# madsjulia/GeostatInversion.jl

Measured on AMD Instinct MI355X. Metric: randSVD GB/s + top-k singular-value rel-err, n=1e6 rank=256, higher is better.
Workload: dtype f64

## Files before the change

### geostatinversion.jl_amd/build.py

```python
import os
import shutil
import subprocess
import sys
from concurrent.futures import ThreadPoolExecutor

HERE = os.path.dirname(os.path.abspath(__file__))
CSRC = os.path.join(HERE, "csrc")
OBJ = os.path.join(HERE, "build")
LIB = os.path.join(HERE, "libgsi_hip.so")
SOURCES = ["gemm_f64.hip", "gemm_f64_gen1.hip", "syrk_f64.hip", "panel_lu_leaf.hip", "panel_lu_blocks.hip", "panel_lu_streamed.hip", "panel_lu_sharded.hip", "panel_qr.hip", "cholqr.hip", "lowrank_power.hip", "jacobi_svd.hip", "misc.hip", "lsqr_dev.hip", "block_cg.hip", "block_pcg.hip", "block_slq.hip", "pivoted_chol.hip", "pointcov_gemm.hip", "fft_cov.hip", "fft_gridcov_plan.hip", "fftrf_sample.hip", "fftrf_interp.hip", "interp_adjoint.hip", "gridcov_sample.hip","pcga_forward.hip", "fwd_adjoint.hip", "chol_saddle.hip", "posterior_var.hip", "posterior_exact.hip",
           "hip_backend.hip", "hip_backend_products.hip", "hip_backend_sampler.hip", "hip_backend_panels.hip", "hip_backend_lowrank.hip", "hip_backend_pcga.hip",
           "hip_comm.hip", "pipeline.cpp", "solvers.cpp", "pcga.cpp", "api.cpp"]
HEADERS = ["backend.hpp", "hip_backend.hpp", "hip_backend_impl.hpp", "hip_common.hpp", "panel_lu_dev.hpp", "pipeline.hpp", "solvers.hpp", "pcga.hpp", "lsqr_state.hpp", "cg_state.hpp", "block_cg_host.hpp", "slq_state.hpp", "pchol_state.hpp", "pivoted_chol_host.hpp", "pointcov.hpp", "pointcov_gen.hpp", "host_staging.hpp", "gemm_f64_kernel.inc.hpp", "fft_line.hpp", "jacobi_sched.hpp", "fwd_plan.hpp", "fwd_adjoint_plan.hpp", "fwd_adjoint_host.hpp", "fftrf_points.hpp", "interp_adjoint_plan.hpp", "saddle_host.hpp", "posterior_host.hpp", "posterior_exact_host.hpp", "../../include/gsi_hip.h"]
CXXFLAGS = ["-O3", "-std=c++17", "-fPIC", "--offload-arch=gfx950", "-Wall", "-Wno-unused-function",
            "-Wno-unused-result", "-Wno-unused-value"]
RESOURCE_FLAG = "-Rpass-analysis=kernel-resource-usage"
_RES_KEYS = {"TotalSGPRs": "sgprs", "VGPRs": "vgprs", "AGPRs": "agprs", "ScratchSize [bytes/lane]": "scratch_bytes_per_lane",
             "Occupancy [waves/SIMD]": "occupancy_waves_per_simd", "SGPRs Spill": "sgpr_spills", "VGPRs Spill": "vgpr_spills",
             "LDS Size [bytes/block]": "lds_bytes_per_block", "Dynamic Stack": "dynamic_stack"}


def parse_resource_remarks(text):
    out, cur = {}, None
    for line in text.splitlines():
        if "remark:" not in line or "[-Rpass-analysis=kernel-resource-usage]" not in line:
            continue
        body = line.split("remark:", 1)[1].replace("[-Rpass-analysis=kernel-resource-usage]", "").strip()
        if ":" not in body:
            continue
        key, val = [x.strip() for x in body.rsplit(":", 1)]
        if key == "Function Name":
            cur = out.setdefault(val, {})
        elif cur is not None and key in _RES_KEYS:
            cur[_RES_KEYS[key]] = (val == "True") if key == "Dynamic Stack" else int(val)
    return out


def hipcc_version():
    r = subprocess.run([_hipcc(), "--version"], capture_output=True, text=True)
    lines = [ln.strip() for ln in r.stdout.splitlines() if ln.strip()]
    return "; ".join(lines[:2])


def kernel_resources():
    import json
    res = {}
    for src in SOURCES:
        if not src.endswith(".hip"):
            continue
        path = os.path.join(OBJ, src.replace(".", "_") + ".resources.json")
        if not os.path.exists(path):
            raise RuntimeError(f"{path} missing: run build() (it recompiles sources whose resource record is absent)")
        for name, r in json.load(open(path)).items():
            res[name] = dict(r, source=src)
    return res


def _hipcc():
    for cand in (shutil.which("hipcc"), "/opt/rocm/bin/hipcc"):
        if cand and os.path.exists(cand):
            return cand
    raise RuntimeError("hipcc not found: libgsi_hip.so cannot be built (there is no CPU fallback)")


def _newer(target, deps):
    if not os.path.exists(target):
# ... 52 lines not shown
```

### geostatinversion.jl_amd/csrc/cholqr.hip

```cpp
#include "hip_common.hpp"
#include <atomic>
#include <cfloat>
#include <cstdio>
#include <cstdlib>

namespace gsi { namespace hipk {

constexpr int CQ_TB = 32;

__global__ __launch_bounds__(256) void cq_diagmax_kernel(const double* __restrict__ G, int l, double* __restrict__ tiny) {
  __shared__ double s[256];
  double mx = 0.0;
  for (int i = threadIdx.x; i < l; i += 256) mx = fmax(mx, G[i + (int64_t)i * l]);
  s[threadIdx.x] = mx;
  __syncthreads();
  for (int st = 128; st > 0; st >>= 1) {
    if (threadIdx.x < st) s[threadIdx.x] = fmax(s[threadIdx.x], s[threadIdx.x + st]);
    __syncthreads();
  }
  if (threadIdx.x == 0) tiny[0] = s[0] * (double)l * DBL_EPSILON * 16.0;
}

__device__ __forceinline__ double cq_bcast(double v, int src) {
  const int lo = __builtin_amdgcn_readlane(__double2loint(v), src);
  const int hi = __builtin_amdgcn_readlane(__double2hiint(v), src);
  return __hiloint2double(hi, lo);
}

__global__ __launch_bounds__(256) void cq_chol_block_kernel(double* __restrict__ G, int l, int j0, int b,
                                                            const double* __restrict__ tiny_p,
                                                            double* __restrict__ Xout ,
                                                            int32_t* __restrict__ flag) {
  __shared__ double X[CQ_TB][CQ_TB + 1];
  const int tid = threadIdx.x;
  if (tid < 64) {
    const double tiny = tiny_p[0];
    const int c = tid & (CQ_TB - 1);
    double col[CQ_TB], x[CQ_TB];
#pragma unroll
    for (int r = 0; r < CQ_TB; ++r)
      col[r] = (r < b && c < b) ? G[(j0 + r) + (int64_t)(j0 + c) * l] : (r == c ? 1.0 : 0.0);
    bool bad = false;
#pragma unroll
    for (int k = 0; k < CQ_TB; ++k) {
      double d = cq_bcast(col[k], k);
      if (k < b && !(d > tiny)) { bad = true; d = 1.0; }
      const double ukk = sqrt(d);
      col[k] = (c == k) ? ukk : col[k] / ukk;
#pragma unroll
      for (int r = k + 1; r < CQ_TB; ++r) col[r] -= cq_bcast(col[k], r) * col[k];
      __builtin_amdgcn_sched_barrier(0);
    }
    if (bad && tid == 0) atomicOr(flag, 1);
#pragma unroll
    for (int r = CQ_TB - 1; r >= 0; --r) {
      double sacc = (r == c) ? 1.0 : 0.0;
#pragma unroll
      for (int p = r + 1; p < CQ_TB; ++p) sacc -= cq_bcast(col[r], p) * x[p];
      x[r] = (r <= c) ? sacc / cq_bcast(col[r], r) : 0.0;
      __builtin_amdgcn_sched_barrier(0);
    }
    if (tid < CQ_TB) {
#pragma unroll
      for (int r = 0; r < CQ_TB; ++r) {
        X[r][c] = x[r];
        Xout[r + c * CQ_TB] = x[r];
        if (r < b && c < b) G[(j0 + r) + (int64_t)(j0 + c) * l] = (r <= c) ? col[r] : 0.0;
      }
    }
  }
  __syncthreads();
  for (int c = j0 + b + tid; c < l; c += 256) {
    double g[CQ_TB];
#pragma unroll
    for (int r = 0; r < CQ_TB; ++r) g[r] = (r < b) ? G[(j0 + r) + (int64_t)c * l] : 0.0;
#pragma unroll 1
    for (int r = 0; r < b; ++r) {
      double s = 0.0;
#pragma unroll
      for (int p = 0; p < CQ_TB; ++p) s += X[p][r] * g[p];
// ... 11 lines not shown
  __shared__ double Xs[CQ_TB][CQ_TB + 1];
  __shared__ double xs[8][CQ_TB + 1];
  const int tid = threadIdx.x, c = tid & (CQ_TB - 1), rl = tid >> 5;
  for (int e = tid; e < CQ_TB * CQ_TB; e += 256) Xs[e & (CQ_TB - 1)][e >> 5] = X[e];
  for (int64_t r0 = (int64_t)blockIdx.x * 8; r0 < m; r0 += (int64_t)gridDim.x * 8) {
    const int64_t r = r0 + rl;
    __syncthreads();
    xs[rl][c] = (r < m && c < b) ? Y[r + (j0 + c) * ld] : 0.0;
    __syncthreads();
    double s = 0.0;
#pragma unroll
    for (int p = 0; p < CQ_TB; ++p) s += xs[rl][p] * Xs[p][c];
    if (r < m && c < b) Y[r + (j0 + c) * ld] = s;
  }
}

__global__ __launch_bounds__(256) void cq_orth_check_kernel(const double* __restrict__ G, int l, double thresh,
                                                            int32_t* __restrict__ flag) {
  const int64_t total = (int64_t)l * l;
  bool bad = false;
  for (int64_t e = (int64_t)blockIdx.x * 256 + threadIdx.x; e < total; e += (int64_t)gridDim.x * 256) {
    const int r = (int)(e % l), c = (int)(e / l);
    const double v = G[e] - (r == c ? 1.0 : 0.0);
    if (!(fabs(v) <= thresh)) bad = true;
  }
  if (bad) atomicOr(flag, 2);
}

__global__ void cq_mirror_upper_kernel(double* __restrict__ G, int l) {
  const int64_t total = (int64_t)l * l;
  for (int64_t e = (int64_t)blockIdx.x * blockDim.x + threadIdx.x; e < total; e += (int64_t)gridDim.x * blockDim.x) {
    const int r = (int)(e % l), c = (int)(e / l);
    if (r > c) G[e] = G[c + (int64_t)r * l];
  }
}

__global__ void cq_triprod_kernel(const double* __restrict__ R2, const double* __restrict__ R1, int l,
                                  double* __restrict__ R) {
  const int64_t total = (int64_t)l * l;
  for (int64_t e = (int64_t)blockIdx.x * blockDim.x + threadIdx.x; e < total;
       e += (int64_t)gridDim.x * blockDim.x) {
    const int r = (int)(e % l), c = (int)(e / l);
    double s = 0.0;
    if (r <= c)
      for (int p = r; p <= c; ++p) s += R2[r + (int64_t)p * l] * R1[p + (int64_t)c * l];
    R[e] = s;
  }
}

constexpr int CQF_THREADS = 512;
constexpr int CQF_MAXL = 384;
constexpr int CQF_LDU = CQF_MAXL - CQ_TB + 16;
constexpr int CQF_LDK = CQF_MAXL - CQ_TB + 4;
constexpr int CQF_DS = CQ_TB + 4;
static_assert(CQF_LDU % 32 == 16 && CQF_LDK % 32 == 4, "LDS strides");
typedef double cq_double4 __attribute__((ext_vector_type(4)));
constexpr size_t CQF_LDS_BYTES = sizeof(double) * ((size_t)CQ_TB * CQF_LDU + (size_t)CQ_TB * CQF_DS + 2 * CQ_TB + 64);

__device__ __forceinline__ void cqf_chol_diag(double* __restrict__ G, int l, int j0, int b, double tiny, double* __restrict__ Ds,
                                                        double* __restrict__ Dinv, int32_t* __restrict__ flag, int lane) {
  const int c = lane & (CQ_TB - 1);
  double col[CQ_TB];
#pragma unroll
  for (int r = 0; r < CQ_TB; ++r)
    col[r] = (r < b && c < b && r <= c) ? G[(j0 + r) + (int64_t)(j0 + c) * l] : (r == c ? 1.0 : 0.0);
  bool bad = false;
  double rdiag = 1.0;
#pragma unroll
  for (int k = 0; k < CQ_TB; ++k) {
    double d = cq_bcast(col[k], k);
    if (k < b && !(d > tiny)) { bad = true; d = 1.0; }
    double rs = __builtin_amdgcn_rsq(d);
    rs = rs * (1.5 - 0.5 * d * rs * rs);
    rs = rs * (1.5 - 0.5 * d * rs * rs);
    const double ukk = d * rs;
    col[k] = (c == k) ? ukk : col[k] * rs;
    if (c == k) rdiag = rs;
#pragma unroll
    for (int r = k + 1; r < CQ_TB; ++r) col[r] -= cq_bcast(col[k], r) * col[k];
    __builtin_amdgcn_sched_barrier(0);
  }
  if (bad && lane == 0) atomicOr(flag, 1);
  if (lane < CQ_TB) {
    Dinv[c] = rdiag;
#pragma unroll
    for (int r = 0; r < CQ_TB; ++r) {
      const double v = (r <= c) ? col[r] : 0.0;
      Ds[r * CQF_DS + c] = v;
      if (r < b && c < b) G[(j0 + r) + (int64_t)(j0 + c) * l] = v;
    }
  }
}
__device__ __forceinline__ void cqf_inv_diag(const double* __restrict__ G, int l, int j0, int b, double* __restrict__ X, int lane) {
  const int c = lane & (CQ_TB - 1);
  double col[CQ_TB], x[CQ_TB];
#pragma unroll
  for (int r = 0; r < CQ_TB; ++r)
    col[r] = (r < b && c < b && r <= c) ? G[(j0 + r) + (int64_t)(j0 + c) * l] : (r == c ? 1.0 : 0.0);
#pragma unroll
  for (int r = CQ_TB - 1; r >= 0; --r) {
    double sacc = (r == c) ? 1.0 : 0.0;
#pragma unroll
    for (int p = r + 1; p < CQ_TB; ++p) sacc -= cq_bcast(col[r], p) * x[p];
    x[r] = (r <= c) ? sacc / cq_bcast(col[r], r) : 0.0;
    __builtin_amdgcn_sched_barrier(0);
  }
  if (lane < CQ_TB && c < b) {
#pragma unroll
    for (int r = 0; r < CQ_TB; ++r)
      if (r < b) X[(j0 + r) + (int64_t)(j0 + c) * l] = x[r];
  }
}
template <bool VEC>
__device__ __forceinline__ void cqf_block_row_col(double* __restrict__ gcol , int b,
                                                  const double* __restrict__ Ds, const double* __restrict__ Dinv,
                                                  double* __restrict__ us ) {
  double g[CQ_TB];
  if constexpr (VEC) {
    const double2* g2 = reinterpret_cast<const double2*>(gcol);
#pragma unroll
    for (int p = 0; p < CQ_TB; p += 2) { const double2 v = g2[p >> 1]; g[p] = v.x; g[p + 1] = v.y; }
  } else {
#pragma unroll
    for (int p = 0; p < CQ_TB; ++p) g[p] = (p < b) ? gcol[p] : 0.0;
  }
#pragma unroll
  for (int pb = 0; pb < CQ_TB; pb += 8) {
    double acc[8];
#pragma unroll
    for (int j = 0; j < 8; ++j) acc[j] = g[pb + j];
#pragma unroll 4
    for (int q = 0; q < pb; ++q) {
      const double uq = us[q * CQF_LDU];
      const double* dr = Ds + q * CQF_DS + pb;
#pragma unroll
      for (int j = 0; j < 8; ++j) acc[j] -= dr[j] * uq;
    }
#pragma unroll
    for (int j = 0; j < 8; ++j) {
#pragma unroll
      for (int i = 0; i < j; ++i) acc[j] -= Ds[(pb + i) * CQF_DS + pb + j] * acc[i];
      acc[j] *= Dinv[pb + j];
    }
#pragma unroll
    for (int j = 0; j < 8; ++j) {
      const double v = (pb + j < b) ? acc[j] : 0.0;
      us[(pb + j) * CQF_LDU] = v;
      if constexpr (!VEC) { if (pb + j < b) gcol[pb + j] = v; }
    }
    if constexpr (VEC) {
      double2* o2 = reinterpret_cast<double2*>(gcol + pb);
#pragma unroll
      for (int j = 0; j < 8; j += 2) o2[j >> 1] = make_double2(acc[j], acc[j + 1]);
    }
    asm volatile("" ::: "memory");
  }
}
#define CQF_STAMP(ph) do { if (trace != nullptr && tid == 0) { const unsigned long long now_ = wall_clock64(); trace[ph] += now_ - t_last; t_last = now_; } } while (0)
__device__ __forceinline__ void cqf_tri_inverse(const double* __restrict__ G, int l, double* __restrict__ X, double* Us,
                                                double* Ds, int tid, int lane, int wave, unsigned long long* trace,
                                                unsigned long long& t_last);
__global__ __launch_bounds__(CQF_THREADS) void cq_chol_inv_kernel(double* __restrict__ G, int l, double* __restrict__ X,
                                                                  int32_t* __restrict__ flag, unsigned long long* __restrict__ trace,
                                                                  const int32_t* __restrict__ skip) {
  if (skip != nullptr && *skip != 0) return;
// ... 337 lines not shown
        phiT = diag ? 0.5 * t : t;
        q = diag ? di * di : accQ[jj] + (di + dJ[wave * CQS_NJ + jj]) * r1;
      }
      const double one = diag ? 1.0 : 0.0;
      rv = (one + r1) - phiT;
      xv = (one - r1) + (q + phiT);
    }
    G[i + (int64_t)j * l] = rv;
    X[i + (int64_t)j * l] = xv;
  }
}

static inline int grid_for(int64_t total, int cap = 2048) {
  int64_t g = (total + 255) / 256;
  if (g > cap) g = cap;
  if (g < 1) g = 1;
  return (int)g;
}

__global__ void cq_identity_kernel(double* __restrict__ X, int l) {
  const int64_t total = (int64_t)l * l;
  for (int64_t e = (int64_t)blockIdx.x * blockDim.x + threadIdx.x; e < total; e += (int64_t)gridDim.x * blockDim.x)
    X[e] = (e % l == e / l) ? 1.0 : 0.0;
}

__global__ __launch_bounds__(256) void cq_shift_kernel(double* __restrict__ G, int l, double m) {
  __shared__ double s[256], mx[256];
  double tr = 0.0, dm = 0.0;
  for (int i = threadIdx.x; i < l; i += 256) {
    const double g = G[i + (int64_t)i * l];
    tr += g;
    dm = fmax(dm, g);
  }
  s[threadIdx.x] = tr;
  mx[threadIdx.x] = dm;
  __syncthreads();
  for (int st = 128; st > 0; st >>= 1) {
    if (threadIdx.x < st) {
      s[threadIdx.x] += s[threadIdx.x + st];
      mx[threadIdx.x] = fmax(mx[threadIdx.x], mx[threadIdx.x + st]);
    }
    __syncthreads();
  }
  const double shift = fmax(4.0 * (double)l * sqrt(m) * (0.5 * DBL_EPSILON) * s[0], 4.0 * 16.0 * (double)l * DBL_EPSILON * mx[0]);
  for (int i = threadIdx.x; i < l; i += 256) G[i + (int64_t)i * l] += shift;
}

size_t cholqr_small_doubles(int64_t l) {
  const int64_t nblk = (l + CQ_TB - 1) / CQ_TB;
  return (size_t)(7 * l * l + nblk * CQ_TB * CQ_TB + 64);
}

namespace {
struct CqBufs { double *R1, *R2, *R3, *Gt, *X1, *X2, *X3, *Rinv; };
inline CqBufs cq_bufs(double* small, int l) {
  const size_t ll = (size_t)l * l;
  return {small, small + ll, small + 2 * ll, small + 3 * ll, small + 4 * ll, small + 5 * ll, small + 6 * ll,
          small + 7 * ll};
}

void cq_round(hipStream_t st, const double* src, int64_t lds, double* dst, int64_t ldd, int64_t m, int l, double* Rp,
              double* X, const CqBufs& b, bool check, int32_t* flag, double* gemm_ws, bool apply, bool shift = false) {
  const int nblk = (l + CQ_TB - 1) / CQ_TB;
  if (!syrk_full_from_upper(st, l, m, src, lds, Rp, l, gemm_ws)) {
    gemm_f64_syrk_upper(st, l, m, src, lds, Rp, l, gemm_ws);
    hipLaunchKernelGGL(cq_mirror_upper_kernel, dim3(64), dim3(256), 0, st, Rp, l);
  }
  if (check)
    hipLaunchKernelGGL(cq_orth_check_kernel, dim3(grid_for((int64_t)l * l, 64)), dim3(256), 0, st, Rp, l, 0.1, flag);
  if (shift) hipLaunchKernelGGL(cq_shift_kernel, dim3(1), dim3(256), 0, st, Rp, l, (double)m);
  static const bool fused_off = (getenv("GSI_CQ_FUSED") != nullptr && getenv("GSI_CQ_FUSED")[0] == '0');
  if (!fused_off && l <= CQF_MAXL && l >= 1) {
    static std::atomic<uint64_t> attr_mask{0};
    if (first_use_on_this_device(attr_mask))
      (void)hipFuncSetAttribute((const void*)cq_chol_inv_kernel, hipFuncAttributeMaxDynamicSharedMemorySize, (int)CQF_LDS_BYTES);
    static const bool trace_on = (getenv("GSI_CQ_TRACE") != nullptr);
    unsigned long long* trace = nullptr;
    if (trace_on && hipMalloc((void**)&trace, 8 * sizeof(unsigned long long)) == hipSuccess) hipMemsetAsync(trace, 0, 8 * sizeof(unsigned long long), st);
    hipLaunchKernelGGL(cq_chol_inv_kernel, dim3(1), dim3(CQF_THREADS), CQF_LDS_BYTES, st, Rp, l, X, flag, trace,
                       (const int32_t*)nullptr);
    if (trace != nullptr) {
      unsigned long long h[8];
      hipMemcpyAsync(h, trace, sizeof(h), hipMemcpyDeviceToHost, st);
      hipStreamSynchronize(st);
      hipFree(trace);
      fprintf(stderr, "[gsi cq trace] l = %d: set-up %.1f us, diagonal blocks %.1f, block rows %.1f, trailing updates %.1f, diagonal inverses %.1f, "
              "W rows %.1f, inverse tiles %.1f\n", l, h[0] / 100.0, h[1] / 100.0, h[2] / 100.0, h[3] / 100.0, h[4] / 100.0, h[5] / 100.0, h[6] / 100.0);
    }
    if (apply && !trmm_upper_tall(st, m, l, src, lds, X, l, dst, ldd))
      gemm_f64_trmm_upper(st, m, l, l, src, lds, X, l, dst, ldd, gemm_ws);
    return;
  }
  hipLaunchKernelGGL(cq_diagmax_kernel, dim3(1), dim3(256), 0, st, Rp, l, b.Gt);
  for (int jb = 0; jb < nblk; ++jb) {
    const int j0 = jb * CQ_TB;
    const int bb = (l - j0 < CQ_TB) ? (l - j0) : CQ_TB;
    hipLaunchKernelGGL(cq_chol_block_kernel, dim3(1), dim3(256), 0, st, Rp, l, j0, bb, b.Gt,
                       b.Rinv + (size_t)jb * CQ_TB * CQ_TB, flag);
    const int t = l - j0 - bb;
    if (t > 0)
      gemm_f64(st, true, t, t, bb, -1.0, Rp + j0 + (int64_t)(j0 + bb) * l, l, Rp + j0 + (int64_t)(j0 + bb) * l, l, 1.0,
               Rp + (j0 + bb) + (int64_t)(j0 + bb) * l, l, gemm_ws);
  }
  hipLaunchKernelGGL(cq_identity_kernel, dim3(grid_for((int64_t)l * l, 256)), dim3(256), 0, st, X, l);
  for (int jb = 0; jb < nblk; ++jb) {
    const int64_t j0 = (int64_t)jb * CQ_TB;
    const int bb = (int)((l - j0 < CQ_TB) ? (l - j0) : CQ_TB);
    if (j0 > 0)
      gemm_f64(st, false, j0 + bb, bb, j0, -1.0, X, l, Rp + j0 * (int64_t)l, l, 1.0, X + j0 * l, l, gemm_ws);
    hipLaunchKernelGGL(cq_right_mult_kernel, dim3((unsigned)((j0 + bb + 7) / 8)), dim3(256), 0, st, X, j0 + bb, (int64_t)l,
                       j0, bb, b.Rinv + (size_t)jb * CQ_TB * CQ_TB);
  }
  if (apply && !trmm_upper_tall(st, m, l, src, lds, X, l, dst, ldd))
    gemm_f64_trmm_upper(st, m, l, l, src, lds, X, l, dst, ldd, gemm_ws);
}
}

void cholqr2_factor(hipStream_t st, const double* Y, int64_t m, int64_t l64, int64_t ld, double* T, int64_t ldt,
                    double* small, int32_t* flag, double* gemm_ws) {
  const int l = (int)l64;
  const CqBufs b = cq_bufs(small, l);
  cq_round(st, Y, ld, T, ldt, m, l, b.R1, b.X1, b, false, flag, gemm_ws, true);
  cq_round(st, T, ldt, nullptr, 0, m, l, b.R2, b.X2, b, true, flag, gemm_ws, false);
}

void cholqr2_apply(hipStream_t st, double* Y, int64_t m, int64_t l64, int64_t ld, const double* T, int64_t ldt,
                   double* R, double* small, double* gemm_ws) {
  const int l = (int)l64;
  const CqBufs b = cq_bufs(small, l);
  if (!trmm_upper_tall(st, m, l, T, ldt, b.X2, l, Y, ld)) gemm_f64_trmm_upper(st, m, l, l, T, ldt, b.X2, l, Y, ld, gemm_ws);
  if (R != nullptr)
    hipLaunchKernelGGL(cq_triprod_kernel, dim3(grid_for((int64_t)l * l, 256)), dim3(256), 0, st, b.R2, b.R1, l, R);
}

void cholqr2_R(hipStream_t st, int64_t l64, double* small, double* R) {
  const int l = (int)l64;
  const CqBufs b = cq_bufs(small, l);
  hipLaunchKernelGGL(cq_triprod_kernel, dim3(grid_for((int64_t)l * l, 256)), dim3(256), 0, st, b.R2, b.R1, l, R);
}
const double* cholqr2_X2(const double* small, int64_t l) { return small + 5 * (size_t)l * (size_t)l; }

void mirror_upper(hipStream_t st, double* G, int64_t l) {
  hipLaunchKernelGGL(cq_mirror_upper_kernel, dim3(64), dim3(256), 0, st, G, (int)l);
}
bool cq_gram_round(hipStream_t st, double* Gm, int64_t l64, double* X, bool check, int32_t* flag, int32_t* series, double* tmp) {
  const int l = (int)l64;
  if (l < 1 || l > CQF_MAXL) return false;
  static const bool series_off = (getenv("GSI_CQ_SERIES") != nullptr && getenv("GSI_CQ_SERIES")[0] == '0');
  const bool by_series = check && !series_off && series != nullptr && tmp != nullptr;
  if (by_series) hipLaunchKernelGGL(cq_mirror_copy_kernel, dim3(64), dim3(256), 0, st, Gm, l, tmp);
  else hipLaunchKernelGGL(cq_mirror_upper_kernel, dim3(64), dim3(256), 0, st, Gm, l);
  if (check)
    hipLaunchKernelGGL(cq_orth_check_kernel, dim3(grid_for((int64_t)l * l, 64)), dim3(256), 0, st, Gm, l, 0.1, flag);
  if (by_series) {
    const int nb = (l + CQS_T - 1) / CQS_T;
    hipLaunchKernelGGL(cq_series_norm_kernel, dim3(1), dim3(CQF_THREADS), 0, st, tmp, l, CQS_GATE, series);
    hipLaunchKernelGGL(cq_series_kernel, dim3(nb * nb), dim3(CQF_THREADS), 0, st, Gm, l, X, tmp, (const int32_t*)series);
  }
  static std::atomic<uint64_t> attr_mask{0};
  if (first_use_on_this_device(attr_mask))
    (void)hipFuncSetAttribute((const void*)cq_chol_inv_kernel, hipFuncAttributeMaxDynamicSharedMemorySize, (int)CQF_LDS_BYTES);
  hipLaunchKernelGGL(cq_chol_inv_kernel, dim3(1), dim3(CQF_THREADS), CQF_LDS_BYTES, st, Gm, l, X, flag,
                     (unsigned long long*)nullptr, by_series ? (const int32_t*)(series + 1) : (const int32_t*)nullptr);
  return true;
}
void tri_product(hipStream_t st, const double* R2, const double* R1, int64_t l, double* R) {
  hipLaunchKernelGGL(cq_triprod_kernel, dim3(grid_for(l * l, 256)), dim3(256), 0, st, R2, R1, (int)l, R);
}

__global__ __launch_bounds__(256) void lr_gather_rows_kernel(const double* __restrict__ S, int64_t lds, int64_t N,
                                                             const int64_t* __restrict__ src, const int64_t* __restrict__ sub,
                                                             int64_t nr, double* __restrict__ R, int64_t ldr) {
  const int64_t total = nr * N;
  for (int64_t e = (int64_t)blockIdx.x * blockDim.x + threadIdx.x; e < total; e += (int64_t)gridDim.x * blockDim.x) {
    const int64_t k = e % nr, c = e / nr;
    const double* col = S + c * lds;
    const int64_t s = sub[k];
    double v = col[src[k]];
    if (s >= 0) v -= col[s];
    R[k + c * ldr] = v;
  }
}
__global__ __launch_bounds__(256) void lr_check_rows_kernel(const double* __restrict__ E, int64_t lde,
                                                            const double* __restrict__ L, int64_t ldl,
                                                            const int64_t* __restrict__ rows, int64_t nchk, int64_t l,
                                                            double* __restrict__ part) {
  __shared__ double red[4];
  double mx = 0.0;
  const int64_t total = nchk * l;
  for (int64_t e = (int64_t)blockIdx.x * blockDim.x + threadIdx.x; e < total; e += (int64_t)gridDim.x * blockDim.x) {
    const int64_t k = e % nchk, j = e / nchk;
    const double d = fabs(E[k + j * lde] - L[rows[k] + j * ldl]);
    if (!(d <= mx)) mx = (d != d) ? INFINITY : d;
  }
  for (int off = 32; off > 0; off >>= 1) mx = fmax(mx, __shfl_xor(mx, off, 64));
  if ((threadIdx.x & 63) == 0) red[threadIdx.x >> 6] = mx;
  __syncthreads();
  if (threadIdx.x == 0) part[blockIdx.x] = fmax(fmax(red[0], red[1]), fmax(red[2], red[3]));
}
bool tri_inverse(hipStream_t st, const double* R, int64_t l64, double* X) {
  const int l = (int)l64;
  if (l < 1 || l > CQF_MAXL) return false;
  static std::atomic<uint64_t> attr_mask{0};
  if (first_use_on_this_device(attr_mask))
    (void)hipFuncSetAttribute((const void*)cq_tri_inv_kernel, hipFuncAttributeMaxDynamicSharedMemorySize, (int)CQF_LDS_BYTES);
  hipLaunchKernelGGL(cq_tri_inv_kernel, dim3(1), dim3(CQF_THREADS), CQF_LDS_BYTES, st, R, l, X);
  return true;
}
void lr_gather_rows(hipStream_t st, const double* S, int64_t lds, int64_t N, const int64_t* src, const int64_t* sub,
                    int64_t nr, double* R, int64_t ldr) {
  if (nr < 1 || N < 1) return;
// ... 30 lines not shown
```

### geostatinversion.jl_amd/csrc/hip_common.hpp

```cpp
#pragma once
#include <hip/hip_runtime.h>
#include <atomic>
#include <cstdint>
#include <cstddef>
#include "pointcov.hpp"

namespace gsi { struct FwdProduct; struct FwdAdjoint; }

namespace gsi { namespace hipk {

inline bool first_use_on_this_device(std::atomic<uint64_t>& mask) {
  int dev = 0;
  if (hipGetDevice(&dev) != hipSuccess || dev < 0 || dev > 63) return true;
  const uint64_t bit = (uint64_t)1 << dev;
  return (mask.fetch_or(bit, std::memory_order_acq_rel) & bit) == 0;
}

struct GemmPlan { int64_t nt, nchunks, xmode, wide, nsplit, persistent, grid_x, active; };
size_t gemm_workspace_doubles(int64_t M, int64_t L, int64_t K);
void gemm_f64(hipStream_t st, bool transA, int64_t M, int64_t L, int64_t K, double alpha, const double* A,
              int64_t lda, const double* B, int64_t ldb, double beta, double* C, int64_t ldc, double* ws,
              GemmPlan* plan = nullptr);
bool gemm_f64_nn_capped(hipStream_t st, int64_t M, int64_t L, int64_t K, const double* A, int64_t lda, const double* B,
                        int64_t ldb, double* C, int64_t ldc, int max_grid, bool query_only = false, GemmPlan* plan = nullptr);
// ... 169 lines not shown

void slq_trace_begin(hipStream_t st, const double* state, double* tr, int64_t qmax);
void slq_trace_step(hipStream_t st, const double* state, double* tr, int64_t qmax);
void slq_quadrature(hipStream_t st, const double* alpha, const double* beta, const double* steps, const double* rho0,
                    int64_t qmax, int64_t b, double* work, double* out);
void slq_sample_rows(hipStream_t st, int64_t n, int64_t b, const double* e, const double* Y, const double* G2, double* Zout);

struct PcholCol {
  int form;
  const double* a;
  int64_t ld;
  int32_t ny;
  int dim, kind;
  double sigma2, nugget;
};
size_t pchol_work_doubles(int form, int64_t n, int64_t K);
double* pchol_points(double* work, int64_t n, int64_t K);
void pchol_begin(hipStream_t st, const PcholCol& a, int64_t n, int64_t K, double tol, const double* L, int64_t ldl, double* d,
                 double* work);
void pchol_step(hipStream_t st, const PcholCol& a, int64_t n, int64_t K, double* L, int64_t ldl, double* d, double* work);
void scale_cols(hipStream_t st, int64_t n, int64_t K, double* U, int64_t ldu, const double* S);

constexpr int QR_NB = 16;
struct QrWork {
  double* coef;
  double* part;
  double* tau;
  double* T;
  double* G;
  double* Vbuf;
  double* Wt;
  double* W2;
  double* Qo;
  int64_t maxblocks;
};
int64_t qr_max_blocks(int64_t m);
void qr_thinQ(hipStream_t st, double* Y, int64_t m, int64_t l, int64_t ld, double* R, const QrWork& w,
              double* gemm_ws);
constexpr int QR_AMAX_PARTS = 256;
void qr_absmax(hipStream_t st, const double* Y, int64_t m, int64_t l, int64_t ld, double* amax_ws);
int qr_prescale_exponent(double amax);
void qr_scale(hipStream_t st, double* A, int64_t rows, int64_t cols, int64_t ld, double s);

size_t cholqr_small_doubles(int64_t l);
void cholqr2_factor(hipStream_t st, const double* Y, int64_t m, int64_t l, int64_t ld, double* T, int64_t ldt,
                    double* small_ws, int32_t* flag, double* gemm_ws);
void cholqr2_apply(hipStream_t st, double* Y, int64_t m, int64_t l, int64_t ld, const double* T, int64_t ldt,
                   double* R, double* small_ws, double* gemm_ws);
void cholqr2_R(hipStream_t st, int64_t l, double* small_ws, double* R);
const double* cholqr2_X2(const double* small_ws, int64_t l);
void mirror_upper(hipStream_t st, double* G, int64_t l);
bool cq_gram_round(hipStream_t st, double* Gm, int64_t l, double* X, bool check, int32_t* flag, int32_t* series = nullptr,
                   double* tmp = nullptr);
void tri_product(hipStream_t st, const double* R2, const double* R1, int64_t l, double* R);
bool tri_inverse(hipStream_t st, const double* R, int64_t l, double* X);
void lr_gather_rows(hipStream_t st, const double* S, int64_t lds, int64_t N, const int64_t* src, const int64_t* sub,
                    int64_t nr, double* R, int64_t ldr);
void lr_check_rows(hipStream_t st, const double* E, int64_t lde, const double* L, int64_t ldl, const int64_t* rows,
                   int64_t nchk, int64_t l, double* part, int nparts);
void scholqr3_factor(hipStream_t st, const double* Y, int64_t m, int64_t l, int64_t ld, double* T, int64_t ldt,
                     double* S, int64_t lds, double* small_ws, int32_t* flag, double* gemm_ws);
void scholqr3_apply(hipStream_t st, double* Y, int64_t m, int64_t l, int64_t ld, const double* S, int64_t lds,
                    double* R, double* small_ws, double* gemm_ws);

void lr_compose(hipStream_t st, const int32_t* piv, const int32_t* info, int64_t n, int64_t l, int64_t nchk, int64_t o_chk,
                int64_t o_sm, int64_t ldr, int64_t* src, int64_t* sub, int64_t* chk, int32_t* verdict);
void lr_solve_u(hipStream_t st, const double* L, int64_t ldl, const double* Mp, int64_t l, double c, double* Ut);
void lr_solve_c(hipStream_t st, const double* Ut, int64_t l, const double* T, int64_t N, double c, double* C);
void lr_solve_u12(hipStream_t st, const double* L, int64_t ldl, const double* Mp, int64_t l1, int64_t l, double c, double* Ut11,
                  double* U12);
void lr_move_rows(hipStream_t st, double* X, int64_t ldx, int64_t nc, const int64_t* src, const int64_t* sub,
                  const int32_t* verdict, int64_t maxmv, double* tmp, int64_t ldt, int64_t nzero);
void lr_pivots(hipStream_t st, const int32_t* piv, int64_t cnt, int64_t add, int32_t* dst);
void lr_forget_zero_pivot(hipStream_t st, int32_t* info);
struct SvdWork {
  int32_t* rotcount;
  double* norms;
  int32_t* pairs;
};
constexpr int SVD_SCHED_INTS = 4096;
int svd_small(hipStream_t st, double* G, int64_t l, double* U, double* S, const SvdWork& w);

void center_rows(hipStream_t st, double* S, int64_t n, int64_t N, int64_t ld);
void scale_cols_sqrt(hipStream_t st, double* U, int64_t l, const double* S, int64_t K);
void randn_fill(hipStream_t st, double* p, size_t count, uint64_t seed);
void fill_gridcov(hipStream_t st, double* A, int64_t lda, int64_t nx, int64_t ny, double ell, int kind,
                  int64_t row0, int64_t mloc);
void fill_lowrank_samples(hipStream_t st, double* S, int64_t ld, int64_t nloc, int64_t N, int64_t row0, uint64_t seed,
                          double decay);
void colnorms_sq(hipStream_t st, const double* Y, int64_t m, int64_t c, int64_t ld, double* out_dev);
void chol_upper(hipStream_t st, double* B, int64_t j, int32_t* info);
void trsm_right_upper(hipStream_t st, double* F, int64_t m, int64_t j, int64_t ldf, const double* C);
void axpy(hipStream_t st, int64_t n, double a, const double* x, double* y);
void scal_copy(hipStream_t st, int64_t n, double a, const double* x, double* y);
void dot_dev(hipStream_t st, int64_t n, const double* x, const double* y, double* out_dev);
void scal(hipStream_t st, int64_t n, double a, double* x);
void gemv_n(hipStream_t st, int64_t m, int64_t k, double alpha, const double* A, int64_t lda, const double* x, double beta,
            double* y);
size_t gemv_t_workspace_doubles(int64_t k);
void gemv_t(hipStream_t st, int64_t m, int64_t k, double alpha, const double* A, int64_t lda, const double* x, double* y,
            double* part);
void project_out(hipStream_t st, int64_t m, int64_t ncols, const double* q, double* Y, int64_t ld, double* part);
void diag_mul_add(hipStream_t st, int64_t n, const double* d, const double* x, double* y);
void f64_to_f32(hipStream_t st, const double* src, float* dst, size_t count);
void pcga_params_f32(hipStream_t st, const float* Z, int64_t n, int64_t K, const double* s, const double* X, double delta,
                     double* out);
// ... 33 lines not shown
```

Baseline: 1794.

## Add multi-workgroup blocked Cholesky and triangular inverse for CholQR Gram factor

Replaces the single-workgroup fused Cholesky+inverse kernel with a sequence of per-block-column launches. Each launch spreads the trailing strip updates and triangular solves across several workgroups using MFMA f64. The triangular inverse then runs as a separate multi-block kernel. The aim is to stop the l×l (l=256) Gram factorization from being serialized on one CU. In exchange it adds about l/32 extra kernel launches and global-memory round trips between steps, and can be disabled through environment variables.

```diff
diff --git a/geostatinversion.jl_amd/build.py b/geostatinversion.jl_amd/build.py
--- a/geostatinversion.jl_amd/build.py
+++ b/geostatinversion.jl_amd/build.py
@@ -8,10 +8,10 @@
 CSRC = os.path.join(HERE, "csrc")
 OBJ = os.path.join(HERE, "build")
 LIB = os.path.join(HERE, "libgsi_hip.so")
-SOURCES = ["gemm_f64.hip", "gemm_f64_gen1.hip", "syrk_f64.hip", "panel_lu_leaf.hip", "panel_lu_blocks.hip", "panel_lu_streamed.hip", "panel_lu_sharded.hip", "panel_qr.hip", "cholqr.hip", "lowrank_power.hip", "jacobi_svd.hip", "misc.hip", "lsqr_dev.hip", "block_cg.hip", "block_pcg.hip", "block_slq.hip", "pivoted_chol.hip", "pointcov_gemm.hip", "fft_cov.hip", "fft_gridcov_plan.hip", "fftrf_sample.hip", "fftrf_interp.hip", "interp_adjoint.hip", "gridcov_sample.hip","pcga_forward.hip", "fwd_adjoint.hip", "chol_saddle.hip", "posterior_var.hip", "posterior_exact.hip",
+SOURCES = ["gemm_f64.hip", "gemm_f64_gen1.hip", "syrk_f64.hip", "panel_lu_leaf.hip", "panel_lu_blocks.hip", "panel_lu_streamed.hip", "panel_lu_sharded.hip", "panel_qr.hip", "cholqr.hip", "chol_blocked_mw.hip", "lowrank_power.hip", "jacobi_svd.hip", "misc.hip", "lsqr_dev.hip", "block_cg.hip", "block_pcg.hip", "block_slq.hip", "pivoted_chol.hip", "pointcov_gemm.hip", "fft_cov.hip", "fft_gridcov_plan.hip", "fftrf_sample.hip", "fftrf_interp.hip", "interp_adjoint.hip", "gridcov_sample.hip","pcga_forward.hip", "fwd_adjoint.hip", "chol_saddle.hip", "posterior_var.hip", "posterior_exact.hip",
            "hip_backend.hip", "hip_backend_products.hip", "hip_backend_sampler.hip", "hip_backend_panels.hip", "hip_backend_lowrank.hip", "hip_backend_pcga.hip",
            "hip_comm.hip", "pipeline.cpp", "solvers.cpp", "pcga.cpp", "api.cpp"]
-HEADERS = ["backend.hpp", "hip_backend.hpp", "hip_backend_impl.hpp", "hip_common.hpp", "panel_lu_dev.hpp", "pipeline.hpp", "solvers.hpp", "pcga.hpp", "lsqr_state.hpp", "cg_state.hpp", "block_cg_host.hpp", "slq_state.hpp", "pchol_state.hpp", "pivoted_chol_host.hpp", "pointcov.hpp", "pointcov_gen.hpp", "host_staging.hpp", "gemm_f64_kernel.inc.hpp", "fft_line.hpp", "jacobi_sched.hpp", "fwd_plan.hpp", "fwd_adjoint_plan.hpp", "fwd_adjoint_host.hpp", "fftrf_points.hpp", "interp_adjoint_plan.hpp", "saddle_host.hpp", "posterior_host.hpp", "posterior_exact_host.hpp", "../../include/gsi_hip.h"]
+HEADERS = ["backend.hpp", "hip_backend.hpp", "hip_backend_impl.hpp", "hip_common.hpp", "panel_lu_dev.hpp", "pipeline.hpp", "solvers.hpp", "pcga.hpp", "lsqr_state.hpp", "cg_state.hpp", "block_cg_host.hpp", "slq_state.hpp", "pchol_state.hpp", "pivoted_chol_host.hpp", "pointcov.hpp", "pointcov_gen.hpp", "host_staging.hpp", "gemm_f64_kernel.inc.hpp", "cholqr_diag.inc.hpp", "fft_line.hpp", "jacobi_sched.hpp", "fwd_plan.hpp", "fwd_adjoint_plan.hpp", "fwd_adjoint_host.hpp", "fftrf_points.hpp", "interp_adjoint_plan.hpp", "saddle_host.hpp", "posterior_host.hpp", "posterior_exact_host.hpp", "../../include/gsi_hip.h"]
 CXXFLAGS = ["-O3", "-std=c++17", "-fPIC", "--offload-arch=gfx950", "-Wall", "-Wno-unused-function",
             "-Wno-unused-result", "-Wno-unused-value"]
 RESOURCE_FLAG = "-Rpass-analysis=kernel-resource-usage"
diff --git a/geostatinversion.jl_amd/csrc/chol_blocked_mw.hip b/geostatinversion.jl_amd/csrc/chol_blocked_mw.hip
--- /dev/null
+++ b/geostatinversion.jl_amd/csrc/chol_blocked_mw.hip
@@ -0,0 +1,282 @@
+#include "hip_common.hpp"
+#include "cholqr_diag.inc.hpp"
+#include <atomic>
+#include <cfloat>
+
+namespace gsi { namespace hipk {
+
+constexpr int CQM_THREADS = 512;
+constexpr int CQM_MAXL = 384;
+constexpr int CQM_LDT = CQ_TB + 1;
+constexpr int CQM_XROWS = CQM_MAXL;
+constexpr int CQM_KC = 64;
+constexpr int CQM_LDK = CQM_KC + 4;
+constexpr int CQM_SB = 4 * (CQM_MAXL / CQ_TB - 1);
+static_assert(CQM_LDK % 32 == 4, "LDS stride");
+
+__device__ __forceinline__ double cqm_load(const double* __restrict__ p, bool ok) { return ok ? *p : 0.0; }
+
+__global__ __launch_bounds__(CQM_THREADS) void cqmw_block_kernel(double* __restrict__ G, int l, int jb, double* __restrict__ X,
+                                                                 int32_t* __restrict__ flag, int nstrips) {
+  constexpr int POOL_A = 2 * CQ_TB * CQM_LDK, POOL_B = 2 * CQ_TB * CQF_DS + 2 * CQ_TB * CQM_LDT;
+  __shared__ double pool[POOL_A > POOL_B ? POOL_A : POOL_B];
+  double* St = pool;
+  double (*Dp)[CQ_TB * CQF_DS] = reinterpret_cast<double (*)[CQ_TB * CQF_DS]>(pool);
+  double (*Tp)[CQ_TB * CQM_LDT] = reinterpret_cast<double (*)[CQ_TB * CQM_LDT]>(pool + 2 * CQ_TB * CQF_DS);
+  __shared__ double Ds[CQ_TB * CQF_DS];
+  __shared__ double Dinv[CQ_TB];
+  __shared__ double red[CQM_THREADS / 64 + 1];
+  const int tid = threadIdx.x, lane = tid & 63;
+  const int wave = __builtin_amdgcn_readfirstlane(tid >> 6);
+  const int nblk = (l + CQ_TB - 1) / CQ_TB;
+  const int j0 = jb * CQ_TB;
+  const int b = (l - j0 < CQ_TB) ? (l - j0) : CQ_TB;
+
+  if (jb > 0 && blockIdx.x == gridDim.x - 1) {
+    const int p0 = j0 - CQ_TB;
+    for (int e = tid; e < CQ_TB * CQ_TB; e += CQM_THREADS) {
+      const int r = e & (CQ_TB - 1), c = e >> 5;
+      const int64_t at = (int64_t)(p0 + r) + (int64_t)(p0 + c) * l;
+      G[at] = (r <= c) ? X[at] : 0.0;
+    }
+    const int nbelow = l - j0;
+    for (int e = tid; e < CQ_TB * nbelow; e += CQM_THREADS) {
+      const int r = j0 + e % nbelow, c = p0 + e / nbelow;
+      G[r + (int64_t)c * l] = 0.0;
+    }
+    __syncthreads();
+    if (wave == 0) cqf_inv_diag(G, l, p0, CQ_TB, X, lane);
+    return;
+  }
+
+  double tiny;
+  if (jb == 0) {
+    double mx = 0.0;
+    for (int i = tid; i < l; i += CQM_THREADS) mx = fmax(mx, G[i + (int64_t)i * l]);
+    for (int off = 32; off > 0; off >>= 1) mx = fmax(mx, __shfl_xor(mx, off, 64));
+    if (lane == 0) red[wave] = mx;
+    __syncthreads();
+    if (tid == 0) {
+      double m2 = 0.0;
+      for (int w2 = 0; w2 < CQM_THREADS / 64; ++w2) m2 = fmax(m2, red[w2]);
+      red[CQM_THREADS / 64] = m2 * (double)l * DBL_EPSILON * 16.0;
+    }
+    __syncthreads();
+    tiny = red[CQM_THREADS / 64];
+    if (nblk > 1 && blockIdx.x == 0 && tid == 0) X[l - 1] = tiny;
+  } else {
+    tiny = X[l - 1];
+  }
+
+  const bool has_strip = (int)blockIdx.x < nstrips;
+  const int c0 = j0 + b + (int)blockIdx.x * CQ_TB;
+  {
+    const int t = wave & 3, kh = wave >> 2, tr = t >> 1, tc = t & 1;
+    const int jl = lane & 15, kq = lane >> 4;
+    const bool doD = (tr <= tc);
+    cq_double4 accD = (cq_double4){0.0, 0.0, 0.0, 0.0}, accT = accD;
+    if (kh == 0) {
+      const int r = tr * 16 + jl;
+#pragma unroll
+      for (int v = 0; v < 4; ++v) {
+        const int c = tc * 16 + kq + 4 * v;
+        accD[v] = cqm_load(G + (int64_t)(j0 + r) + (int64_t)(j0 + c) * l, doD && r < b && c < b);
+        accT[v] = cqm_load(G + (int64_t)(j0 + r) + (int64_t)(c0 + c) * l, has_strip && r < b && c0 + c < l);
+      }
+    }
+    const int scol = tid >> 3, sk = tid & 7;
+    const int gcol = (scol < CQ_TB) ? j0 + scol : c0 + scol - CQ_TB;
+    const bool scol_ok = gcol < l && (scol < CQ_TB || has_strip);
+    const double* sp = G + (int64_t)(scol_ok ? gcol : 0) * l + sk;
+    double sv[8];
+    auto fetch = [&](int k0) __attribute__((always_inline)) {
+#pragma unroll
+      for (int u = 0; u < 8; ++u) sv[u] = cqm_load(sp + (k0 + 8 * u < j0 ? k0 + 8 * u : 0), scol_ok && k0 + sk + 8 * u < j0);
+    };
+    if (j0 > 0) fetch(0);
+    for (int k0 = 0; k0 < j0; k0 += CQM_KC) {
+      __syncthreads();
+#pragma unroll
+      for (int u = 0; u < 8; ++u) St[scol * CQM_LDK + sk + 8 * u] = sv[u];
+      __syncthreads();
+      if (k0 + CQM_KC < j0) fetch(k0 + CQM_KC);
+      const double* sd = St + (tc * 16 + jl) * CQM_LDK + kh * (CQM_KC / 2) + kq;
+      const double* sr = St + (tr * 16 + jl) * CQM_LDK + kh * (CQM_KC / 2) + kq;
+      const double* stt = St + (CQ_TB + tc * 16 + jl) * CQM_LDK + kh * (CQM_KC / 2) + kq;
+#pragma unroll
+      for (int st4 = 0; st4 < CQM_KC / 8; ++st4) {
+        const double fr = sr[4 * st4];
+        if (doD) accD = __builtin_amdgcn_mfma_f64_16x16x4f64(-sd[4 * st4], fr, accD, 0, 0, 0);
+        accT = __builtin_amdgcn_mfma_f64_16x16x4f64(-stt[4 * st4], fr, accT, 0, 0, 0);
+      }
+    }
+    __syncthreads();
+    const int r = tr * 16 + jl;
+#pragma unroll
+    for (int v = 0; v < 4; ++v) {
+      const int c = tc * 16 + kq + 4 * v;
+      Dp[kh][c * CQF_DS + r] = accD[v];
+      Tp[kh][c * CQM_LDT + r] = accT[v];
+    }
+  }
+  __syncthreads();
+  for (int e = tid; e < CQ_TB * CQ_TB; e += CQM_THREADS) {
+    const int r = e & (CQ_TB - 1), c = e >> 5;
+    Dp[0][c * CQF_DS + r] += Dp[1][c * CQF_DS + r];
+    Tp[0][c * CQM_LDT + r] += Tp[1][c * CQM_LDT + r];
+  }
+  __syncthreads();
+  if (wave == 0) cqf_chol_diag(Dp[0], CQF_DS, 0, b, tiny, Ds, Dinv, flag, lane);
+  __syncthreads();
+  if (blockIdx.x == 0) {
+    for (int e = tid; e < CQ_TB * CQ_TB; e += CQM_THREADS) {
+      const int r = e & (CQ_TB - 1), c = e >> 5;
+      if (r < b && c < b) X[(int64_t)(j0 + r) + (int64_t)(j0 + c) * l] = Ds[r * CQF_DS + c];
+    }
+  }
+  if (!has_strip) return;
+  if (tid < CQ_TB && c0 + tid < l) {
+    double* tcol = Tp[0] + tid * CQM_LDT;
+    double g[CQ_TB];
+#pragma unroll
+    for (int p = 0; p < CQ_TB; ++p) g[p] = (p < b) ? tcol[p] : 0.0;
+#pragma unroll
+    for (int pb = 0; pb < CQ_TB; pb += 8) {
+      double acc[8];
+#pragma unroll
+      for (int j = 0; j < 8; ++j) acc[j] = g[pb + j];
+#pragma unroll 4
+      for (int q = 0; q < pb; ++q) {
+        const double uq = tcol[q];
+        const double* dr = Ds + q * CQF_DS + pb;
+#pragma unroll
+        for (int j = 0; j < 8; ++j) acc[j] -= dr[j] * uq;
+      }
+#pragma unroll
+      for (int j = 0; j < 8; ++j) {
+#pragma unroll
+        for (int i = 0; i < j; ++i) acc[j] -= Ds[(pb + i) * CQF_DS + pb + j] * acc[i];
+        acc[j] *= Dinv[pb + j];
+      }
+#pragma unroll
+      for (int j = 0; j < 8; ++j) tcol[pb + j] = (pb + j < b) ? acc[j] : 0.0;
+      asm volatile("" ::: "memory");
+    }
+  }
+  __syncthreads();
+  for (int e = tid; e < CQ_TB * CQ_TB; e += CQM_THREADS) {
+    const int r = e & (CQ_TB - 1), c = e >> 5;
+    if (r < b && c0 + c < l) G[(int64_t)(j0 + r) + (int64_t)(c0 + c) * l] = Tp[0][c * CQM_LDT + r];
+  }
+}
+
+__global__ __launch_bounds__(CQM_THREADS) void cqmw_inverse_kernel(double* __restrict__ G, int l, double* __restrict__ X) {
+  extern __shared__ double cqm_lds[];
+  const int tid = threadIdx.x, lane = tid & 63;
+  const int wave = __builtin_amdgcn_readfirstlane(tid >> 6);
+  const int nblk = (l + CQ_TB - 1) / CQ_TB;
+  const int j = blockIdx.x, j0 = j * CQ_TB;
+  const int b = (l - j0 < CQ_TB) ? (l - j0) : CQ_TB;
+  double* Xs = cqm_lds;
+  double* Sp = Xs + (size_t)nblk * CQ_TB * CQF_DS;
+  if (j == nblk - 1) {
+    for (int e = tid; e < CQ_TB * CQ_TB; e += CQM_THREADS) {
+      const int r = e & (CQ_TB - 1), c = e >> 5;
+      if (r < b && c < b) {
+        const int64_t at = (int64_t)(j0 + r) + (int64_t)(j0 + c) * l;
+        G[at] = (r <= c) ? X[at] : 0.0;
+      }
+    }
+    __syncthreads();
+    if (wave == 0) cqf_inv_diag(G, l, j0, b, X, lane);
+    __syncthreads();
+  }
+  {
+    const int nbelow = l - j0 - b;
+    for (int e = tid; e < b * nbelow; e += CQM_THREADS) {
+      const int r = j0 + b + e % nbelow, c = j0 + e / nbelow;
+      X[r + (int64_t)c * l] = 0.0;
+    }
+  }
+  for (int e = tid; e < CQ_TB * CQ_TB; e += CQM_THREADS) {
+    const int r = e & (CQ_TB - 1), c = e >> 5;
+    Xs[(j0 + r) * CQF_DS + c] = (r < b && c < b) ? X[(int64_t)(j0 + r) + (int64_t)(j0 + c) * l] : 0.0;
+  }
+  __syncthreads();
+  const int t = wave & 3, kh = wave >> 2, tr = t >> 1, tc = t & 1;
+  const int jl = lane & 15, kq = lane >> 4;
+  double fbn[CQM_SB], xb[8] = {0.0, 0.0, 0.0, 0.0, 0.0, 0.0, 0.0, 0.0};
+  auto fetch_u = [&](int i) __attribute__((always_inline)) {
+    const int nst = 4 * (j - i), kbeg = i * CQ_TB + CQ_TB + kh * 4 * nst;
+    const double* up = G + (int64_t)(i * CQ_TB + tr * 16 + jl);
+#pragma unroll
+    for (int u = 0; u < CQM_SB; ++u) {
+      const int k = kbeg + 4 * u + kq;
+      const bool in = u < nst && k < l;
+      fbn[u] = cqm_load(up + (int64_t)(in ? k : 0) * l, in);
+    }
+  };
+  auto fetch_x = [&](int i) __attribute__((always_inline)) {
+    if (kh == 0) {
+#pragma unroll
+      for (int s8 = 0; s8 < 8; ++s8) xb[s8] = X[(int64_t)(i * CQ_TB + tr * 16 + jl) + (int64_t)(i * CQ_TB + 4 * s8 + kq) * l];
+    }
+  };
+  if (j > 0) { fetch_x(j - 1); fetch_u(j - 1); }
+  for (int i = j - 1; i >= 0; --i) {
+    const int i0 = i * CQ_TB;
+    const int nst = 4 * (j - i);
+    const int kbeg = i0 + CQ_TB + kh * 4 * nst;
+    cq_double4 a0 = (cq_double4){0.0, 0.0, 0.0, 0.0}, a1 = a0;
+#pragma unroll
+    for (int u = 0; u < CQM_SB; u += 2) {
+      if (u < nst) {
+        a0 = __builtin_amdgcn_mfma_f64_16x16x4f64(Xs[(kbeg + 4 * u + kq) * CQF_DS + tc * 16 + jl], fbn[u], a0, 0, 0, 0);
+        a1 = __builtin_amdgcn_mfma_f64_16x16x4f64(Xs[(kbeg + 4 * u + 4 + kq) * CQF_DS + tc * 16 + jl], fbn[u + 1], a1, 0, 0, 0);
+      }
+    }
+    const cq_double4 acc = a0 + a1;
+    if (i > 0) fetch_u(i - 1);
+#pragma unroll
+    for (int v = 0; v < 4; ++v) Sp[kh * CQ_TB * CQF_DS + (tr * 16 + jl) * CQF_DS + tc * 16 + kq + 4 * v] = acc[v];
+    __syncthreads();
+    if (kh == 0) {
+      cq_double4 xa = (cq_double4){0.0, 0.0, 0.0, 0.0};
+#pragma unroll
+      for (int s8 = 0; s8 < 8; ++s8) {
+        const int at = (4 * s8 + kq) * CQF_DS + tc * 16 + jl;
+        const double fa = -(Sp[at] + Sp[CQ_TB * CQF_DS + at]);
+        xa = __builtin_amdgcn_mfma_f64_16x16x4f64(fa, xb[s8], xa, 0, 0, 0);
+      }
+#pragma unroll
+      for (int v = 0; v < 4; ++v) {
+        const int r = tr * 16 + jl, c = tc * 16 + kq + 4 * v;
+        Xs[(i0 + r) * CQF_DS + c] = xa[v];
+        if (c < b) X[(int64_t)(i0 + r) + (int64_t)(j0 + c) * l] = xa[v];
+      }
+    }
+    if (i > 0) fetch_x(i - 1);
+    __syncthreads();
+  }
+}
+
+bool chol_inv_mw(hipStream_t st, double* G, int l, double* X, int32_t* flag) {
+  if (l < 1 || l > CQM_MAXL) return false;
+  const int nblk = (l + CQ_TB - 1) / CQ_TB;
+  const size_t lds = sizeof(double) * ((size_t)nblk * CQ_TB * CQF_DS + 2 * (size_t)CQ_TB * CQF_DS);
+  static std::atomic<uint64_t> attr_mask{0};
+  if (first_use_on_this_device(attr_mask))
+    (void)hipFuncSetAttribute((const void*)cqmw_inverse_kernel, hipFuncAttributeMaxDynamicSharedMemorySize,
+                              (int)(sizeof(double) * ((size_t)CQM_XROWS * CQF_DS + 2 * (size_t)CQ_TB * CQF_DS)));
+  for (int jb = 0; jb < nblk; ++jb) {
+    const int j0 = jb * CQ_TB;
+    const int b = (l - j0 < CQ_TB) ? (l - j0) : CQ_TB;
+    const int nstrips = (l - j0 - b + CQ_TB - 1) / CQ_TB;
+    const int grid = (nstrips > 0 ? nstrips : 1) + (jb > 0 ? 1 : 0);
+    hipLaunchKernelGGL(cqmw_block_kernel, dim3(grid), dim3(CQM_THREADS), 0, st, G, l, jb, X, flag, nstrips);
+  }
+  hipLaunchKernelGGL(cqmw_inverse_kernel, dim3(nblk), dim3(CQM_THREADS), lds, st, G, l, X);
+  return true;
+}
+
+}}
diff --git a/geostatinversion.jl_amd/csrc/cholqr.hip b/geostatinversion.jl_amd/csrc/cholqr.hip
--- a/geostatinversion.jl_amd/csrc/cholqr.hip
+++ b/geostatinversion.jl_amd/csrc/cholqr.hip
@@ -1,4 +1,5 @@
 #include "hip_common.hpp"
+#include "cholqr_diag.inc.hpp"
 #include <atomic>
 #include <cfloat>
 #include <cstdio>
@@ -6,7 +7,6 @@
 
 namespace gsi { namespace hipk {
 
-constexpr int CQ_TB = 32;
 
 __global__ __launch_bounds__(256) void cq_diagmax_kernel(const double* __restrict__ G, int l, double* __restrict__ tiny) {
   __shared__ double s[256];
@@ -21,11 +21,6 @@
   if (threadIdx.x == 0) tiny[0] = s[0] * (double)l * DBL_EPSILON * 16.0;
 }
 
-__device__ __forceinline__ double cq_bcast(double v, int src) {
-  const int lo = __builtin_amdgcn_readlane(__double2loint(v), src);
-  const int hi = __builtin_amdgcn_readlane(__double2hiint(v), src);
-  return __hiloint2double(hi, lo);
-}
 
 __global__ __launch_bounds__(256) void cq_chol_block_kernel(double* __restrict__ G, int l, int j0, int b,
                                                             const double* __restrict__ tiny_p,
@@ -143,65 +138,9 @@
 constexpr int CQF_MAXL = 384;
 constexpr int CQF_LDU = CQF_MAXL - CQ_TB + 16;
 constexpr int CQF_LDK = CQF_MAXL - CQ_TB + 4;
-constexpr int CQF_DS = CQ_TB + 4;
 static_assert(CQF_LDU % 32 == 16 && CQF_LDK % 32 == 4, "LDS strides");
-typedef double cq_double4 __attribute__((ext_vector_type(4)));
 constexpr size_t CQF_LDS_BYTES = sizeof(double) * ((size_t)CQ_TB * CQF_LDU + (size_t)CQ_TB * CQF_DS + 2 * CQ_TB + 64);
 
-__device__ __forceinline__ void cqf_chol_diag(double* __restrict__ G, int l, int j0, int b, double tiny, double* __restrict__ Ds,
-                                                        double* __restrict__ Dinv, int32_t* __restrict__ flag, int lane) {
-  const int c = lane & (CQ_TB - 1);
-  double col[CQ_TB];
-#pragma unroll
-  for (int r = 0; r < CQ_TB; ++r)
-    col[r] = (r < b && c < b && r <= c) ? G[(j0 + r) + (int64_t)(j0 + c) * l] : (r == c ? 1.0 : 0.0);
-  bool bad = false;
-  double rdiag = 1.0;
-#pragma unroll
-  for (int k = 0; k < CQ_TB; ++k) {
-    double d = cq_bcast(col[k], k);
-    if (k < b && !(d > tiny)) { bad = true; d = 1.0; }
-    double rs = __builtin_amdgcn_rsq(d);
-    rs = rs * (1.5 - 0.5 * d * rs * rs);
-    rs = rs * (1.5 - 0.5 * d * rs * rs);
-    const double ukk = d * rs;
-    col[k] = (c == k) ? ukk : col[k] * rs;
-    if (c == k) rdiag = rs;
-#pragma unroll
-    for (int r = k + 1; r < CQ_TB; ++r) col[r] -= cq_bcast(col[k], r) * col[k];
-    __builtin_amdgcn_sched_barrier(0);
-  }
-  if (bad && lane == 0) atomicOr(flag, 1);
-  if (lane < CQ_TB) {
-    Dinv[c] = rdiag;
-#pragma unroll
-    for (int r = 0; r < CQ_TB; ++r) {
-      const double v = (r <= c) ? col[r] : 0.0;
-      Ds[r * CQF_DS + c] = v;
-      if (r < b && c < b) G[(j0 + r) + (int64_t)(j0 + c) * l] = v;
-    }
-  }
-}
-__device__ __forceinline__ void cqf_inv_diag(const double* __restrict__ G, int l, int j0, int b, double* __restrict__ X, int lane) {
-  const int c = lane & (CQ_TB - 1);
-  double col[CQ_TB], x[CQ_TB];
-#pragma unroll
-  for (int r = 0; r < CQ_TB; ++r)
-    col[r] = (r < b && c < b && r <= c) ? G[(j0 + r) + (int64_t)(j0 + c) * l] : (r == c ? 1.0 : 0.0);
-#pragma unroll
-  for (int r = CQ_TB - 1; r >= 0; --r) {
-    double sacc = (r == c) ? 1.0 : 0.0;
-#pragma unroll
-    for (int p = r + 1; p < CQ_TB; ++p) sacc -= cq_bcast(col[r], p) * x[p];
-    x[r] = (r <= c) ? sacc / cq_bcast(col[r], r) : 0.0;
-    __builtin_amdgcn_sched_barrier(0);
-  }
-  if (lane < CQ_TB && c < b) {
-#pragma unroll
-    for (int r = 0; r < CQ_TB; ++r)
-      if (r < b) X[(j0 + r) + (int64_t)(j0 + c) * l] = x[r];
-  }
-}
 template <bool VEC>
 __device__ __forceinline__ void cqf_block_row_col(double* __restrict__ gcol , int b,
                                                   const double* __restrict__ Ds, const double* __restrict__ Dinv,
@@ -645,6 +584,12 @@
 }
 
 namespace {
+constexpr int CQMW_MIN = 64;
+inline bool cq_mw_wanted(int l) {
+  static const bool off = (getenv("GSI_CQ_MW") != nullptr && getenv("GSI_CQ_MW")[0] == '0');
+  static const int lo = (getenv("GSI_CQ_MW_MIN") != nullptr && atoi(getenv("GSI_CQ_MW_MIN")) >= 1) ? atoi(getenv("GSI_CQ_MW_MIN")) : CQMW_MIN;
+  return !off && l >= lo && l <= CQF_MAXL;
+}
 struct CqBufs { double *R1, *R2, *R3, *Gt, *X1, *X2, *X3, *Rinv; };
 inline CqBufs cq_bufs(double* small, int l) {
   const size_t ll = (size_t)l * l;
@@ -668,6 +613,11 @@
     if (first_use_on_this_device(attr_mask))
       (void)hipFuncSetAttribute((const void*)cq_chol_inv_kernel, hipFuncAttributeMaxDynamicSharedMemorySize, (int)CQF_LDS_BYTES);
     static const bool trace_on = (getenv("GSI_CQ_TRACE") != nullptr);
+    if (!trace_on && cq_mw_wanted(l) && chol_inv_mw(st, Rp, l, X, flag)) {
+      if (apply && !trmm_upper_tall(st, m, l, src, lds, X, l, dst, ldd))
+        gemm_f64_trmm_upper(st, m, l, l, src, lds, X, l, dst, ldd, gemm_ws);
+      return;
+    }
     unsigned long long* trace = nullptr;
     if (trace_on && hipMalloc((void**)&trace, 8 * sizeof(unsigned long long)) == hipSuccess) hipMemsetAsync(trace, 0, 8 * sizeof(unsigned long long), st);
     hipLaunchKernelGGL(cq_chol_inv_kernel, dim3(1), dim3(CQF_THREADS), CQF_LDS_BYTES, st, Rp, l, X, flag, trace,
@@ -750,6 +700,7 @@
     hipLaunchKernelGGL(cq_series_norm_kernel, dim3(1), dim3(CQF_THREADS), 0, st, tmp, l, CQS_GATE, series);
     hipLaunchKernelGGL(cq_series_kernel, dim3(nb * nb), dim3(CQF_THREADS), 0, st, Gm, l, X, tmp, (const int32_t*)series);
   }
+  if (!check && cq_mw_wanted(l) && chol_inv_mw(st, Gm, l, X, flag)) return true;
   static std::atomic<uint64_t> attr_mask{0};
   if (first_use_on_this_device(attr_mask))
     (void)hipFuncSetAttribute((const void*)cq_chol_inv_kernel, hipFuncAttributeMaxDynamicSharedMemorySize, (int)CQF_LDS_BYTES);
diff --git a/geostatinversion.jl_amd/csrc/cholqr_diag.inc.hpp b/geostatinversion.jl_amd/csrc/cholqr_diag.inc.hpp
--- /dev/null
+++ b/geostatinversion.jl_amd/csrc/cholqr_diag.inc.hpp
@@ -0,0 +1,71 @@
+#pragma once
+#include "hip_common.hpp"
+
+namespace gsi { namespace hipk {
+
+constexpr int CQ_TB = 32;
+constexpr int CQF_DS = CQ_TB + 4;
+typedef double cq_double4 __attribute__((ext_vector_type(4)));
+
+__device__ __forceinline__ double cq_bcast(double v, int src) {
+  const int lo = __builtin_amdgcn_readlane(__double2loint(v), src);
+  const int hi = __builtin_amdgcn_readlane(__double2hiint(v), src);
+  return __hiloint2double(hi, lo);
+}
+
+__device__ __forceinline__ void cqf_chol_diag(double* __restrict__ G, int l, int j0, int b, double tiny, double* __restrict__ Ds,
+                                                        double* __restrict__ Dinv, int32_t* __restrict__ flag, int lane) {
+  const int c = lane & (CQ_TB - 1);
+  double col[CQ_TB];
+#pragma unroll
+  for (int r = 0; r < CQ_TB; ++r)
+    col[r] = (r < b && c < b && r <= c) ? G[(j0 + r) + (int64_t)(j0 + c) * l] : (r == c ? 1.0 : 0.0);
+  bool bad = false;
+  double rdiag = 1.0;
+#pragma unroll
+  for (int k = 0; k < CQ_TB; ++k) {
+    double d = cq_bcast(col[k], k);
+    if (k < b && !(d > tiny)) { bad = true; d = 1.0; }
+    double rs = __builtin_amdgcn_rsq(d);
+    rs = rs * (1.5 - 0.5 * d * rs * rs);
+    rs = rs * (1.5 - 0.5 * d * rs * rs);
+    const double ukk = d * rs;
+    col[k] = (c == k) ? ukk : col[k] * rs;
+    if (c == k) rdiag = rs;
+#pragma unroll
+    for (int r = k + 1; r < CQ_TB; ++r) col[r] -= cq_bcast(col[k], r) * col[k];
+    __builtin_amdgcn_sched_barrier(0);
+  }
+  if (bad && lane == 0) atomicOr(flag, 1);
+  if (lane < CQ_TB) {
+    Dinv[c] = rdiag;
+#pragma unroll
+    for (int r = 0; r < CQ_TB; ++r) {
+      const double v = (r <= c) ? col[r] : 0.0;
+      Ds[r * CQF_DS + c] = v;
+      if (r < b && c < b) G[(j0 + r) + (int64_t)(j0 + c) * l] = v;
+    }
+  }
+}
+__device__ __forceinline__ void cqf_inv_diag(const double* __restrict__ G, int l, int j0, int b, double* __restrict__ X, int lane) {
+  const int c = lane & (CQ_TB - 1);
+  double col[CQ_TB], x[CQ_TB];
+#pragma unroll
+  for (int r = 0; r < CQ_TB; ++r)
+    col[r] = (r < b && c < b && r <= c) ? G[(j0 + r) + (int64_t)(j0 + c) * l] : (r == c ? 1.0 : 0.0);
+#pragma unroll
+  for (int r = CQ_TB - 1; r >= 0; --r) {
+    double sacc = (r == c) ? 1.0 : 0.0;
+#pragma unroll
+    for (int p = r + 1; p < CQ_TB; ++p) sacc -= cq_bcast(col[r], p) * x[p];
+    x[r] = (r <= c) ? sacc / cq_bcast(col[r], r) : 0.0;
+    __builtin_amdgcn_sched_barrier(0);
+  }
+  if (lane < CQ_TB && c < b) {
+#pragma unroll
+    for (int r = 0; r < CQ_TB; ++r)
+      if (r < b) X[(j0 + r) + (int64_t)(j0 + c) * l] = x[r];
+  }
+}
+
+}}
diff --git a/geostatinversion.jl_amd/csrc/hip_common.hpp b/geostatinversion.jl_amd/csrc/hip_common.hpp
--- a/geostatinversion.jl_amd/csrc/hip_common.hpp
+++ b/geostatinversion.jl_amd/csrc/hip_common.hpp
@@ -245,6 +245,7 @@
 void mirror_upper(hipStream_t st, double* G, int64_t l);
 bool cq_gram_round(hipStream_t st, double* Gm, int64_t l, double* X, bool check, int32_t* flag, int32_t* series = nullptr,
                    double* tmp = nullptr);
+bool chol_inv_mw(hipStream_t st, double* G, int l, double* X, int32_t* flag);
 void tri_product(hipStream_t st, const double* R2, const double* R1, int64_t l, double* R);
 bool tri_inverse(hipStream_t st, const double* R, int64_t l, double* X);
 void lr_gather_rows(hipStream_t st, const double* S, int64_t lds, int64_t N, const int64_t* src, const int64_t* sub,
```

After: 1784. No clear change (-0.6%).
